# jasonkyuyim/se3_diffusion

Measured on AMD Instinct MI355X. Metric: residues/sec IPA fwd+bwd, higher is better.
Workload: dtype f32

## Files before the change

include/fd_hip.h:

```cpp
#ifndef FD_HIP_H_
#define FD_HIP_H_

#ifdef __cplusplus
extern "C" {
#endif

#define FD_ABI_VERSION 2

const char* fd_last_error(void);
int fd_abi_version(void);
const char* fd_backend(void);
const char* fd_build_flags(void);
long fd_launch_count(void);

typedef struct FdGemmDesc {
  const float* A;
  const float* B;
  float* C;
  int M, N, K;
  long a_rs, a_cs;
  long b_rs, b_cs;
  long ldc;
  int batch, bdiv;
  long a_so, a_si, b_so, b_si, c_so, c_si;
  float alpha;
  int beta;
  const float* bias;
  const float* pair_p;
  const float* pair_q;
  long ld_pair;
  int nres;
  const float* resid;
  long ld_resid;
  const float* gate;
  long ld_gate;
  const float* rowscale;
  int relu;
  int tile;
  int ksplit;
  int mtiles;
  float* a_rowsum;
  const void* b_planes;
  long b_plane_stride;
} FdGemmDesc;

int fd_gemm(const FdGemmDesc* desc, void* stream);
int fd_split_planes(const float* x, long n, void* planes, void* stream);
int fd_gemm_plan(const FdGemmDesc* desc);
int fd_gemm_set_exact_f32(int exact);
int fd_gemm_set_persistent_blocks(int blocks);

int fd_layernorm_fwd(const float* x, long ldx, const float* gamma, const float* beta, const float* rowscale,
                     float* y, long ldy, float* mean, float* rstd, long rows, int C, float eps, void* stream);
int fd_layernorm_bwd(const float* dy, long lddy, const float* x, long ldx, const float* gamma,
                     const float* rowscale, const float* mean, const float* rstd, float* dx, long lddx,
                     int dx_accum, float* dgamma, float* dbeta, long rows, int C, void* stream);
int fd_colsum_acc(const float* X, long ld, long rows, int ncols, float* out, void* stream);
int fd_pair_reduce_acc(const float* X, int nbatch, int n, int C, float* rowsum, float* colsum, long ld_out,
                       void* stream);
int fd_axpby(float* y, const float* x, float a, float b, long n, void* stream);
int fd_add2d(float* dst, long ldd, const float* src, long lds, long rows, int cols, float a, void* stream);
int fd_rowscale(const float* x, long ldx, const float* rs, float* y, long ldy, long rows, int C, void* stream);

#define FD_EDGE_MLP_IMAGE_BYTES (124 * 12288)
int fd_edge_mlp_pack_zb(const float* W40, void* image, void* stream);
int fd_edge_mlp_pack(const float* W1, const float* W2, const float* Wf, long ld, void* image, void* stream);
int fd_edge_mlp_pack_bwd(const float* Wf, const float* W2, const float* W1, long ld, const float* W40, void* image, void* stream);
typedef struct FdEdgeMlpDesc {
  const float* x;
  const void* img;
  const float* p1;
  const float* q1;
  const float* bias2;
  float* save1;
  float* save2;
  const float* pf;
  const float* qf;
  const float* gamma;
  const float* beta;
  const float* rowscale;
  float* y;
  float* mean;
  float* rstd;
  float* out;
  long rows;
  int nres;
  int backward;
  float eps;
  int blocks;
  long ld_pq;
  long ld_pqf;
  float* zb_out;
  const float* zb_bias;
  unsigned* mask1;
  unsigned* mask2;
  const unsigned* gmask1;
  const unsigned* gmask2;
  const float* ln_y;
  const float* ln_mean;
  const float* ln_rstd;
  const float* ln_gamma;
  const float* ln_rowscale;
  float* dy_out;
  float* ln_dgamma;
  float* ln_dbeta;
  const float* dzb;
  unsigned* sched;
  int shape;
} FdEdgeMlpDesc;
#define FD_EDGE_MLP_W8_MIN_ROWS 65536L
#define FD_EDGE_MLP_PAIR_MAX_ROWS 16384L
int fd_edge_mlp(const FdEdgeMlpDesc* desc, void* stream);

#define FD_EDGE_EMBED_IMAGE_BYTES (24 * 12288)
int fd_edge_embed_pack_zb(const float* W40, void* image, void* stream);
int fd_edge_embed_pack(const float* W0, const float* W2, const float* W4, void* image, void* stream);
typedef struct FdEdgeEmbedDesc {
  const long* seq_idx;
  const float* sc_ca;
  const float* idenom;
  const float* dg_lower;
  const float* dg_upper;
  const void* img;
  const float* p;
  const float* q;
  const float* bias2;
  const float* bias3;
  const float* gamma;
  const float* beta;
  const float* rowscale;
  float* h1;
  float* h2;
  float* h3;
  float* mean;
  float* rstd;
  float* out;
  long rows;
  int nres;
  float eps;
  int blocks;
  float* zb_out;
  const float* zb_bias;
// ... 361 lines not shown
```

se3_diffusion_amd/csrc/fd_norm.hip:

```cpp
#include "fd_common.h"
#include "../../include/fd_hip.h"

namespace {

constexpr int MAXC_PER_LANE = 8;

__global__ __launch_bounds__(256) void layernorm_fwd_kernel(
    const float* __restrict__ x, long ldx, const float* __restrict__ gamma, const float* __restrict__ beta,
    const float* __restrict__ rowscale, float* __restrict__ y, long ldy, float* __restrict__ mean_out,
    float* __restrict__ rstd_out, long rows, int C, float eps) {
  const int lane = fd::lane_id(), wave = fd::wave_id();
  const int npl = C / 64;
  for (long row = (long)blockIdx.x * 4 + wave; row < rows; row += (long)gridDim.x * 4) {
    const float* xr = x + row * ldx;
    float v[MAXC_PER_LANE], gm[MAXC_PER_LANE], bt[MAXC_PER_LANE];
    float s = 0.f;
#pragma unroll
    for (int k = 0; k < MAXC_PER_LANE; ++k)
      if (k < npl) { v[k] = xr[lane + 64 * k]; s += v[k]; }
    const float rs = rowscale ? rowscale[row] : 1.f;
#pragma unroll
    for (int k = 0; k < MAXC_PER_LANE; ++k)
      if (k < npl) { gm[k] = gamma[lane + 64 * k]; bt[k] = beta[lane + 64 * k]; }
    const float mean = fd::wave_sum(s) / (float)C;
// ... 246 lines not shown
    }
#pragma unroll
    for (int u = 0; u < LN_U; ++u) {
      const bool ok = row0 + u < rows;
      const float sc = ok ? rs[u] : 0.f;
      const float4 d = make_float4(dv[u].x * sc, dv[u].y * sc, dv[u].z * sc, dv[u].w * sc);
      const float4 xh = make_float4((xv[u].x - m[u]) * rr[u], (xv[u].y - m[u]) * rr[u], (xv[u].z - m[u]) * rr[u],
                                    (xv[u].w - m[u]) * rr[u]);
      const float4 g = make_float4(d.x * gm.x, d.y * gm.y, d.z * gm.z, d.w * gm.w);
      ag.x += d.x * xh.x; ag.y += d.y * xh.y; ag.z += d.z * xh.z; ag.w += d.w * xh.w;
      ab.x += d.x; ab.y += d.y; ab.z += d.z; ab.w += d.w;
      const float s1 = half_wave_sum((g.x + g.y) + (g.z + g.w)) * (1.0f / 128.0f);
      const float s2 = half_wave_sum((g.x * xh.x + g.y * xh.y) + (g.z * xh.z + g.w * xh.w)) * (1.0f / 128.0f);
      if (ok) {
        float4 o;
        o.x = rr[u] * (g.x - s1 - xh.x * s2);
        o.y = rr[u] * (g.y - s1 - xh.y * s2);
        o.z = rr[u] * (g.z - s1 - xh.z * s2);
        o.w = rr[u] * (g.w - s1 - xh.w * s2);
        if (dx_accum) { o.x += old[u].x; o.y += old[u].y; o.z += old[u].z; o.w += old[u].w; }
        *reinterpret_cast<float4*>(dx + (row0 + u) * lddx + 4 * hl) = o;
      }
    }
  }
  if (dgamma) {
    red[0][wave * 2 + half][hl] = ag;
    red[1][wave * 2 + half][hl] = ab;
    __syncthreads();
    const int t = (int)threadIdx.x;
    const int w = t >> 7, ch = t & 127;
    const float* r0 = reinterpret_cast<const float*>(&red[w][0][0]);
    float a = 0.f;
#pragma unroll
    for (int k = 0; k < 8; ++k) a += r0[k * 128 + ch];
    atomicAdd((w == 0 ? dgamma : dbeta) + ch, a);
  }
}

__global__ __launch_bounds__(256) void colsum_kernel(const float* __restrict__ X, long ld, long rows, int ncols,
                                                      float* __restrict__ out) {
  __shared__ float red[4][64];
  const int lane = fd::lane_id(), wave = fd::wave_id();
  for (int c0 = 0; c0 < ncols; c0 += 64) {
    const int c = c0 + lane;
    float acc = 0.f;
    if (c < ncols)
      for (long r = (long)blockIdx.x * 4 + wave; r < rows; r += (long)gridDim.x * 4) acc += X[r * ld + c];
    red[wave][lane] = acc;
    __syncthreads();
    if (wave == 0 && c < ncols) atomicAdd(&out[c], red[0][lane] + red[1][lane] + red[2][lane] + red[3][lane]);
    __syncthreads();
  }
}

__global__ __launch_bounds__(256) void pair_reduce_kernel(const float* __restrict__ X, int n, int C,
                                                          float* __restrict__ rowsum, float* __restrict__ colsum,
                                                          long ld_out) {
  const long bi = blockIdx.x;
  const long b = bi / n;
  const float* xb = X + bi * (long)n * C;
  for (int c = (int)threadIdx.x; c < C; c += (int)blockDim.x) {
    float acc = 0.f;
    for (int j = 0; j < n; ++j) {
      float v = xb[(long)j * C + c];
      acc += v;
      if (colsum) atomicAdd(&colsum[(b * n + j) * ld_out + c], v);
    }
    if (rowsum) rowsum[bi * ld_out + c] += acc;
  }
}

__global__ __launch_bounds__(256) void pair_colsum_kernel(const float* __restrict__ X, int n, int C,
                                                          float* __restrict__ colsum, long ld_out) {
  const long bj = blockIdx.x;
  const long b = bj / n, j = bj % n;
  const float* xb = X + (b * n * (long)n + j) * C;
  for (int c = (int)threadIdx.x; c < C; c += (int)blockDim.x) {
    float acc = 0.f;
    for (int i = 0; i < n; ++i) acc += xb[(long)i * n * C + c];
    colsum[bj * ld_out + c] += acc;
  }
}

constexpr int PR_I = 32, PR_J = 128, PR_C = 32;
__global__ __launch_bounds__(256) void pair_reduce2_kernel(const float* __restrict__ X, int n, int C,
                                                           float* __restrict__ rowsum, float* __restrict__ colsum,
                                                           long ld_out, int nich, int ncc) {
  __shared__ float4 red[PR_I][4][8];
  const int tid = (int)threadIdx.x;
  const int c4 = tid & 7, jg = tid >> 3, wave = tid >> 6;
  int bx = (int)blockIdx.x;
  const int cc = bx % ncc; bx /= ncc;
  const int ic = bx % nich;
  const long b = bx / nich;
  const int j0 = (int)blockIdx.y * PR_J;
  const int c = cc * PR_C + 4 * c4;
  const int i0 = ic * PR_I;
  float4 cs[PR_J / 32];
#pragma unroll
  for (int q = 0; q < PR_J / 32; ++q) cs[q] = make_float4(0.f, 0.f, 0.f, 0.f);
#pragma unroll 4
  for (int il = 0; il < PR_I; ++il) {
    const int i = i0 + il;
    float4 rs = make_float4(0.f, 0.f, 0.f, 0.f);
    if (i < n) {
      const float* xi = X + ((b * n + i) * (long)n) * C + c;
#pragma unroll
      for (int q = 0; q < PR_J / 32; ++q) {
        const int j = j0 + jg + 32 * q;
        if (j < n) {
          const float4 v = *reinterpret_cast<const float4*>(xi + (long)j * C);
          rs.x += v.x; rs.y += v.y; rs.z += v.z; rs.w += v.w;
          cs[q].x += v.x; cs[q].y += v.y; cs[q].z += v.z; cs[q].w += v.w;
        }
      }
    }
    rs.x += fd::lane_xor8(rs.x); rs.y += fd::lane_xor8(rs.y); rs.z += fd::lane_xor8(rs.z); rs.w += fd::lane_xor8(rs.w);
#pragma unroll
    for (int o = 16; o < 64; o <<= 1) {
      rs.x += __shfl_xor(rs.x, o); rs.y += __shfl_xor(rs.y, o); rs.z += __shfl_xor(rs.z, o); rs.w += __shfl_xor(rs.w, o);
    }
    if ((tid & 63) < 8) red[il][wave][c4] = rs;
  }
#pragma unroll
  for (int q = 0; q < PR_J / 32; ++q) {
    const int j = j0 + jg + 32 * q;
    if (j < n) {
      float* o = colsum + (b * n + j) * ld_out + c;
      atomicAdd(o + 0, cs[q].x); atomicAdd(o + 1, cs[q].y); atomicAdd(o + 2, cs[q].z); atomicAdd(o + 3, cs[q].w);
    }
  }
  __syncthreads();
  {
    const int il = tid >> 3, g = tid & 7;
    const int i = i0 + il;
    if (i < n) {
      float4 a = red[il][0][g];
#pragma unroll
      for (int k = 1; k < 4; ++k) {
        const float4 v = red[il][k][g];
        a.x += v.x; a.y += v.y; a.z += v.z; a.w += v.w;
      }
      float* o = rowsum + (b * n + i) * ld_out + cc * PR_C + 4 * g;
      if (gridDim.y == 1) {
        o[0] += a.x; o[1] += a.y; o[2] += a.z; o[3] += a.w;
      } else {
        atomicAdd(o + 0, a.x); atomicAdd(o + 1, a.y); atomicAdd(o + 2, a.z); atomicAdd(o + 3, a.w);
      }
    }
  }
}

__global__ __launch_bounds__(256) void axpby_kernel(float* __restrict__ y, const float* __restrict__ x, float a,
                                                    float b, long n) {
  for (long i = (long)blockIdx.x * 256 + threadIdx.x; i < n; i += (long)gridDim.x * 256) y[i] = a * x[i] + b * y[i];
}

__global__ __launch_bounds__(256) void rowscale_kernel(const float* __restrict__ x, long ldx,
                                                       const float* __restrict__ rs, float* __restrict__ y, long ldy,
                                                       long rows, int C) {
  const long total = rows * C;
  for (long i = (long)blockIdx.x * 256 + threadIdx.x; i < total; i += (long)gridDim.x * 256) {
    long r = i / C;
    int c = (int)(i % C);
    y[r * ldy + c] = x[r * ldx + c] * rs[r];
  }
}

__global__ __launch_bounds__(256) void colsum4_kernel(const float* __restrict__ X, long ld, long rows, int ncols,
                                                       float* __restrict__ out) {
  __shared__ float4 red[4][64];
  const int lane = fd::lane_id(), wave = fd::wave_id();
  const long wg = (long)blockIdx.x * 4 + wave, nw = (long)gridDim.x * 4;
  for (int c0 = 0; c0 < ncols; c0 += 256) {
    const int c = c0 + lane * 4;
    float4 acc0 = make_float4(0.f, 0.f, 0.f, 0.f), acc1 = acc0, acc2 = acc0, acc3 = acc0;
    if (c < ncols) {
      long r = wg;
      for (; r + 3 * nw < rows; r += 4 * nw) {
        const float4 v0 = *reinterpret_cast<const float4*>(X + r * ld + c);
        const float4 v1 = *reinterpret_cast<const float4*>(X + (r + nw) * ld + c);
        const float4 v2 = *reinterpret_cast<const float4*>(X + (r + 2 * nw) * ld + c);
        const float4 v3 = *reinterpret_cast<const float4*>(X + (r + 3 * nw) * ld + c);
        acc0.x += v0.x; acc0.y += v0.y; acc0.z += v0.z; acc0.w += v0.w;
        acc1.x += v1.x; acc1.y += v1.y; acc1.z += v1.z; acc1.w += v1.w;
        acc2.x += v2.x; acc2.y += v2.y; acc2.z += v2.z; acc2.w += v2.w;
        acc3.x += v3.x; acc3.y += v3.y; acc3.z += v3.z; acc3.w += v3.w;
      }
      for (; r < rows; r += nw) {
        const float4 v0 = *reinterpret_cast<const float4*>(X + r * ld + c);
        acc0.x += v0.x; acc0.y += v0.y; acc0.z += v0.z; acc0.w += v0.w;
      }
    }
    float4 s;
    s.x = (acc0.x + acc1.x) + (acc2.x + acc3.x);
    s.y = (acc0.y + acc1.y) + (acc2.y + acc3.y);
    s.z = (acc0.z + acc1.z) + (acc2.z + acc3.z);
    s.w = (acc0.w + acc1.w) + (acc2.w + acc3.w);
    red[wave][lane] = s;
    __syncthreads();
    {
      const int t = (int)threadIdx.x, cc = c0 + t;
      if (cc < ncols) {
        const float* r0 = reinterpret_cast<const float*>(&red[0][0]);
        atomicAdd(&out[cc], (r0[t] + r0[256 + t]) + (r0[512 + t] + r0[768 + t]));
      }
    }
    __syncthreads();
  }
}

__global__ __launch_bounds__(256) void add2d_kernel(float* __restrict__ dst, long ldd, const float* __restrict__ src,
                                                    long lds, long rows, int cols, float a) {
  const long total = rows * cols;
  for (long i = (long)blockIdx.x * 256 + threadIdx.x; i < total; i += (long)gridDim.x * 256) {
    long r = i / cols;
    int c = (int)(i % cols);
    dst[r * ldd + c] += a * src[r * lds + c];
  }
}

}

static int ln_grid(long rows) {
  long g = (rows + 3) / 4;
  return (int)(g < 1 ? 1 : (g > 8192 ? 8192 : g));
}

static bool ln128_ok(const float* p, long ld) { return fd_aligned16(p) && (ld & 3) == 0; }

extern "C" int fd_layernorm_fwd(const float* x, long ldx, const float* gamma, const float* beta,
                                const float* rowscale, float* y, long ldy, float* mean, float* rstd, long rows,
                                int C, float eps, void* stream) {
  FD_CHECK_ARG(C % 64 == 0 && C <= 64 * MAXC_PER_LANE, "fd_layernorm_fwd: C=%d must be a multiple of 64 <= 512", C);
  if (rows == 0) return FD_OK;
  if (C == 128 && ln128_ok(x, ldx) && ln128_ok(y, ldy) && fd_aligned16(gamma) && fd_aligned16(beta)) {
    long g = (rows + 8 * LN_U - 1) / (8 * LN_U);
    int grid = (int)(g < 1 ? 1 : (g > 4096 ? 4096 : g));
    hipLaunchKernelGGL(layernorm_fwd128_kernel, dim3(grid), dim3(256), 0, (hipStream_t)stream, x, ldx, gamma, beta,
                       rowscale, y, ldy, mean, rstd, rows, eps);
    FD_CHECK_LAUNCH("fd_layernorm_fwd(128)");
    return FD_OK;
  }
  hipLaunchKernelGGL(layernorm_fwd_kernel, dim3(ln_grid(rows)), dim3(256), 0, (hipStream_t)stream, x, ldx, gamma,
                     beta, rowscale, y, ldy, mean, rstd, rows, C, eps);
  FD_CHECK_LAUNCH("fd_layernorm_fwd");
  return FD_OK;
}

extern "C" int fd_layernorm_bwd(const float* dy, long lddy, const float* x, long ldx, const float* gamma,
                                const float* rowscale, const float* mean, const float* rstd, float* dx, long lddx,
                                int dx_accum, float* dgamma, float* dbeta, long rows, int C, void* stream) {
  FD_CHECK_ARG(C % 64 == 0 && C <= 64 * MAXC_PER_LANE, "fd_layernorm_bwd: C=%d must be a multiple of 64 <= 512", C);
  FD_CHECK_ARG((dgamma == nullptr) == (dbeta == nullptr), "fd_layernorm_bwd: dgamma/dbeta come together");
  if (rows == 0) return FD_OK;
  if (C == 128 && ln128_ok(x, ldx) && ln128_ok(dy, lddy) && ln128_ok(dx, lddx) && fd_aligned16(gamma)) {
    long g128 = (rows + 8 * LN_U - 1) / (8 * LN_U);
    int grid128 = (int)(g128 < 1 ? 1 : (g128 > 512 ? 512 : g128));
    hipLaunchKernelGGL(layernorm_bwd128_kernel, dim3(grid128), dim3(256), 0, (hipStream_t)stream, dy, lddy, x, ldx,
                       gamma, rowscale, mean, rstd, dx, lddx, dx_accum, dgamma, dbeta, rows);
    FD_CHECK_LAUNCH("fd_layernorm_bwd(128)");
    return FD_OK;
  }
  long g = (rows + 15) / 16;
  int grid = (int)(g < 1 ? 1 : (g > 1024 ? 1024 : g));
  if (ln128_ok(x, ldx) && ln128_ok(dy, lddy) && ln128_ok(dx, lddx) && fd_aligned16(gamma)) {
    if (C <= 256)
      hipLaunchKernelGGL(layernorm_bwd4_kernel<1>, dim3(grid), dim3(256), 0, (hipStream_t)stream, dy, lddy, x, ldx, gamma,
                         rowscale, mean, rstd, dx, lddx, dx_accum, dgamma, dbeta, rows, C);
    else
      hipLaunchKernelGGL(layernorm_bwd4_kernel<2>, dim3(grid), dim3(256), 0, (hipStream_t)stream, dy, lddy, x, ldx, gamma,
                         rowscale, mean, rstd, dx, lddx, dx_accum, dgamma, dbeta, rows, C);
    FD_CHECK_LAUNCH("fd_layernorm_bwd(x4)");
    return FD_OK;
  }
  hipLaunchKernelGGL(layernorm_bwd_kernel, dim3(grid), dim3(256), 0, (hipStream_t)stream, dy, lddy, x, ldx, gamma,
                     rowscale, mean, rstd, dx, lddx, dx_accum, dgamma, dbeta, rows, C);
  FD_CHECK_LAUNCH("fd_layernorm_bwd");
  return FD_OK;
}

extern "C" int fd_colsum_acc(const float* X, long ld, long rows, int ncols, float* out, void* stream) {
  if (rows == 0 || ncols == 0) return FD_OK;
  long g = (rows + 15) / 16;
  int grid = (int)(g < 1 ? 1 : (g > 1024 ? 1024 : g));
  if ((ld & 3) == 0 && (ncols & 3) == 0 && fd_aligned16(X)) {
    hipLaunchKernelGGL(colsum4_kernel, dim3(grid), dim3(256), 0, (hipStream_t)stream, X, ld, rows, ncols, out);
    FD_CHECK_LAUNCH("fd_colsum_acc");
    return FD_OK;
  }
  hipLaunchKernelGGL(colsum_kernel, dim3(grid), dim3(256), 0, (hipStream_t)stream, X, ld, rows, ncols, out);
  FD_CHECK_LAUNCH("fd_colsum_acc");
  return FD_OK;
}

extern "C" int fd_pair_reduce_acc(const float* X, int nbatch, int n, int C, float* rowsum, float* colsum,
                                  long ld_out, void* stream) {
  if (nbatch == 0 || n == 0) return FD_OK;
  if (rowsum && colsum && (C % PR_C) == 0 && fd_aligned16(X)) {
    const int nich = fd_cdiv(n, PR_I), ncc = C / PR_C;
    hipLaunchKernelGGL(pair_reduce2_kernel, dim3(nbatch * nich * ncc, fd_cdiv(n, PR_J)), dim3(256), 0, (hipStream_t)stream,
                       X, n, C, rowsum, colsum, ld_out, nich, ncc);
    FD_CHECK_LAUNCH("fd_pair_reduce_acc(fused)");
    return FD_OK;
  }
  int threads = C >= 256 ? 256 : (C >= 128 ? 128 : 64);
  if (rowsum) {
    hipLaunchKernelGGL(pair_reduce_kernel, dim3(nbatch * n), dim3(threads), 0, (hipStream_t)stream, X, n, C, rowsum,
                       (float*)nullptr, ld_out);
    FD_CHECK_LAUNCH("fd_pair_reduce_acc(row)");
  }
  if (colsum) {
    hipLaunchKernelGGL(pair_colsum_kernel, dim3(nbatch * n), dim3(threads), 0, (hipStream_t)stream, X, n, C, colsum,
                       ld_out);
    FD_CHECK_LAUNCH("fd_pair_reduce_acc(col)");
  }
  return FD_OK;
}

extern "C" int fd_axpby(float* y, const float* x, float a, float b, long n, void* stream) {
  if (n == 0) return FD_OK;
  long g = (n + 255) / 256;
  int grid = (int)(g > 4096 ? 4096 : g);
  hipLaunchKernelGGL(axpby_kernel, dim3(grid), dim3(256), 0, (hipStream_t)stream, y, x, a, b, n);
  FD_CHECK_LAUNCH("fd_axpby");
  return FD_OK;
}

extern "C" int fd_rowscale(const float* x, long ldx, const float* rs, float* y, long ldy, long rows, int C,
                           void* stream) {
  if (rows == 0 || C == 0) return FD_OK;
  long g = (rows * C + 255) / 256;
  int grid = (int)(g > 4096 ? 4096 : g);
  hipLaunchKernelGGL(rowscale_kernel, dim3(grid), dim3(256), 0, (hipStream_t)stream, x, ldx, rs, y, ldy, rows, C);
  FD_CHECK_LAUNCH("fd_rowscale");
  return FD_OK;
}

extern "C" int fd_add2d(float* dst, long ldd, const float* src, long lds, long rows, int cols, float a,
                        void* stream) {
  if (rows == 0 || cols == 0) return FD_OK;
  long g = (rows * cols + 255) / 256;
  int grid = (int)(g > 4096 ? 4096 : g);
  hipLaunchKernelGGL(add2d_kernel, dim3(grid), dim3(256), 0, (hipStream_t)stream, dst, ldd, src, lds, rows, cols, a);
  FD_CHECK_LAUNCH("fd_add2d");
  return FD_OK;
}
```

se3_diffusion_amd/hip.py:

```python
from __future__ import annotations

import ctypes
import os
from ctypes import POINTER, Structure, c_char_p, c_double, c_float, c_int, c_long, c_void_p

import torch

_HERE = os.path.dirname(os.path.abspath(__file__))
LIB_PATH = os.path.join(_HERE, "lib", "libfd_hip.so")


_RAW_STREAM = getattr(torch._C, "_cuda_getCurrentRawStream", None)


class FdError(RuntimeError):
    pass


class FdGemmDesc(Structure):
    _fields_ = [
        ("A", c_void_p), ("B", c_void_p), ("C", c_void_p),
        ("M", c_int), ("N", c_int), ("K", c_int),
        ("a_rs", c_long), ("a_cs", c_long),
        ("b_rs", c_long), ("b_cs", c_long),
# ... 112 lines not shown


class FdPairDwDesc(Structure):
    _fields_ = [("item", FdPairDwItem * PAIR_DW_MAX_ITEMS), ("nitems", c_int), ("rows", c_long), ("blocks", c_int)]


GROUP_DW_MAX_ITEMS = 32


class FdGroupDwItem(Structure):
    __slots__ = ()
    _fields_ = [("A", c_void_p), ("B", c_void_p), ("C", c_void_p), ("a_colsum", c_void_p),
                ("lda", c_int), ("ldb", c_int), ("ldc", c_int), ("n_out", c_int), ("k_in", c_int)]


class FdGroupDwDesc(Structure):
    _fields_ = [("item", FdGroupDwItem * GROUP_DW_MAX_ITEMS), ("nitems", c_int), ("rows", c_long), ("blocks", c_int)]


OPT_WS_DOUBLES = 3 * 4096
OPT_STATE_BYTES = 72


class FdOptState(Structure):
    __slots__ = ()
    _fields_ = [
        ("step", c_long), ("skipped", c_long), ("clipped", c_long), ("nonfinite", c_long),
        ("grad_norm", c_double), ("clip_coef", c_double), ("max_abs", c_double),
        ("bc1", c_float), ("rsqrt_bc2", c_float), ("coef", c_float), ("apply", c_int),
    ]


assert ctypes.sizeof(FdOptState) == OPT_STATE_BYTES


ABI_VERSION = 2


def _ptr(t, off=0):
    if t is None:
        return None
    if isinstance(t, tuple):
        t, off = t
    return t.data_ptr() + t.element_size() * int(off)


def fill_ptrs(desc, **fields):
    tens = []
    for name, t in fields.items():
        if t is None:
            continue
        if type(t) is tuple:
            off = t[1]
            t = t[0]
            setattr(desc, name, t.data_ptr() + t.element_size() * int(off))
        else:
            setattr(desc, name, t.data_ptr())
        tens.append(t)
    return tens


_SIGS = {
    "fd_gemm": "Ss",
    "fd_gemm_plan": "S",
    "fd_split_planes": "plps",
    "fd_gemm_set_exact_f32": "i",
    "fd_gemm_set_persistent_blocks": "i",
    "fd_edge_mlp_pack": "ppplps",
    "fd_edge_mlp": "Ss",
    "fd_edge_mlp_pack_zb": "pps",
    "fd_edge_mlp_pack_bwd": "ppplpps",
    "fd_edge_embed_pack": "pppps",
    "fd_edge_embed": "Ss",
    "fd_edge_embed_pack_zb": "pps",
    "fd_edge_embed_bwd_pack": "ppps",
    "fd_edge_embed_bwd": "Ss",
    "fd_ln_gemm": "Ss",
    "fd_pair_dw": "Ss",
    "fd_group_dw": "Ss",
    "fd_layernorm_fwd": "plpppplpplifs",
    "fd_layernorm_bwd": "plplpppppl" + "ipplis",
    "fd_colsum_acc": "pllips",
    "fd_pair_reduce_acc": "piiippls",
    "fd_axpby": "ppffls",
    "fd_rowscale": "plppllis",
    "fd_add2d": "plpllifs",
    "fd_node_feats": "ppppppiis",
    "fd_node_feats_ld": "ppppppliis",
    "fd_edge_feats": "pppppppppiis",
    "fd_ipa_points_fwd": "pppppppiliiiis",
    "fd_ipa_points_bwd": "pppppppliiiis",
    "fd_ipa_softmax_fwd": "ppppppiis",
    "fd_ipa_attn_fwd": "ppppppppiis",
    "fd_ipa_flash_fwd": "ppppppppppp" + "iiis",
    "fd_ipa_flash_fwd_split": "ppppppppppp" + "iiii" + "ps",
    "fd_ipa_flash_bwd": "pppppppppppp" + "pppppp" + "iis",
    "fd_ipa_flash_bwd_keys": "pppppppp" + "ppp" + "iiis",
    "fd_ipa_opt_bwd_dot": "ppppppp" + "ls",
    "fd_seq_attn_fwd": "ppppfiis",
    "fd_seq_attn_bwd": "pppppfiis",
    "fd_ipa_attn_bwd": "pppppppppppppiis",
    "fd_ipa_softmax_bwd": "ppppppppppiis",
    "fd_ipa_kpts_bwd": "pppppiis",
    "fd_ipa_dz_acc": "ppplis",
    "fd_ipa_opt_fwd": "ppppls",
    "fd_ipa_opt_bwd": "pppppls",
    "fd_ipa_opair_fwd": "pppiis",
    "fd_ipa_opair_bwd": "pppppiis",
    "fd_row_softmax_fwd": "pplii" + "s",
    "fd_row_softmax_bwd": "pplis",
    "fd_split_rigids": "pfpfppplis",
    "fd_bb_update_fwd": "plipppppppp" + "ls",
    "fd_bb_update_bwd": "pppppppppp" + "ls",
    "fd_heads_fwd": "pppp" + "pl" + "ppp" + "pi" + "S" + "ppppppp" + "iis",
    "fd_heads_bwd": "ppppp" + "ppp" + "pi" + "S" + "ppppp" + "ppp" + "iis",
    "fd_backbone_atoms": "ppSppls",
    "fd_igso3_tables": "ppiiippps",
    "fd_sample_ref": "pppppidpls",
    "fd_forward_marginal": "ppppppipdddipppp" + "ls",
    "fd_forward_marginal_batch": "ppppppippdipppp" + "iis",
    "fd_se3_reverse_step": "ppppppiiddpdddiiips",
    "fd_se3_reverse_step_f32": "ppppppiiddpdddiiips",
    "fd_se3_reverse_step_net": "ppppppiiddpdddiiips",
    "fd_sample_advance": "ppppilpipps",
    "fd_sample_record": "ppppp" + "S" + "piili" + "pppp" + "s",
    "fd_dsm_loss": "Ss",
    "fd_adam_step": "pppplffffffs",
    "fd_adam_step_ema": "ppppplfffffffs",
    "fd_grad_stats": "plpps",
    "fd_adam_step_guarded": "pppplddddd" + "i" + "pp" + "s",
    "fd_adam_step_guarded_ema": "ppppplddddd" + "i" + "pp" + "di" + "s",
    "fd_backbone_metrics": "plpiips",
    "fd_aligned_rmsd": "plplpppiipps",
    "fd_tm_search": "plplppp" + "iiiii" + "ppp" + "s",
    "fd_tm_align": "pliplipppp" + "iiii" + "pppp" + "s",
    "fd_dssp_hbonds": "plppiipps",
    "fd_dssp_assign": "plipppiipps",
    "fd_violations": "plppiippppps",
    "fd_cluster_linkage": "pllp" + "iiii" + "ppps",
    "fd_cluster_cut": "pppllp" + "iii" + "d" + "ppps",
    "fd_chain_windows": "pppips",
    "fd_chain_batch": "pppppp" + "ii" + "S" + "ppppp" + "s",
    "fd_mpnn_graph": "pppp" + "li" + "ppp" + "s",
    "fd_mpnn_encoder": "ppp" + "li" + "pp" + "ppppp" + "s",
    "fd_mpnn_decode": "pp" + "ilii" + "pppp" + "pppppp" + "fi" + "pppp" + "s",
    "fd_pdb_count": "plpp" + "ii" + "pp" + "s",
    "fd_pdb_format": "plppp" + "iil" + "pl" + "s",
}
_CT = {"p": c_void_p, "i": c_int, "l": c_long, "f": c_float, "d": c_double, "S": c_void_p, "s": c_void_p}


class FdLib:

    def __init__(self, path: str):
        if not os.path.exists(path):
            raise FdError(
                f"HIP extension not found at {path}. Build it with "
                f"`python -m se3_diffusion_amd.build` (hipcc, gfx950). There is no CPU fallback.")
        self.path = path
        self.cdll = ctypes.CDLL(path)
        for name, (res, args) in {"fd_last_error": (c_char_p, []), "fd_abi_version": (c_int, []), "fd_launch_count": (c_long, []),
                                  "fd_backend": (c_char_p, []), "fd_build_flags": (c_char_p, [])}.items():
            fn = getattr(self.cdll, name)
            fn.restype, fn.argtypes = res, args
        for name, sig in _SIGS.items():
            fn = getattr(self.cdll, name)
# ... 131 lines not shown
```

se3_diffusion_amd/trunk.py:

```python
from __future__ import annotations

import math

import numpy as np
import torch

from . import hip, ops
from .trace import rng
from . import network as nw
from .network import CS, CZ, TD, H, _lin_grads
from .ops import empty, zeros, mv, lib
from .options import opts

EH = 384
CE = 128


def bb_update_fwd(P, b, n3, dmask, quat, trans, R):
    pre = f"score_model.trunk.bb_update_{b}.linear"
    dev = n3
    upd = empty((R, 6), dev); q2 = empty((R, 4), dev); t2 = empty((R, 3), dev)
    lib().call("fd_bb_update_fwd", n3, CS, CS, dmask, P[f"{pre}.weight"], P[f"{pre}.bias"], quat, trans, upd, q2, t2, R)
    return q2, t2, dict(n3=n3, dmask=dmask, quat=quat, upd=upd, R=R)

# ... 48 lines not shown
        key = ("et_fold", pre)
        if key not in cache:
            Wi, bi = P[f"{pre}.initial_embed.weight"], P[f"{pre}.initial_embed.bias"]
            Wcat = torch.cat([W1[:, CZ:CZ + CE], W1[:, CZ + CE:], Wf[:, CZ:CZ + CE], Wf[:, CZ + CE:]], 0).contiguous()
            Wfold = empty((LDT, CS), Wi)
            ops.linear(mv(Wcat), mv(Wi.t().contiguous()), None, mv(Wfold), LDT, CS, CE)
            bvec = torch.cat([torch.zeros_like(P[f"{pre}.trunk.0.bias"]), P[f"{pre}.trunk.0.bias"],
                              torch.zeros_like(P[f"{pre}.final_layer.bias"]), P[f"{pre}.final_layer.bias"]]).contiguous()
            bfold = empty((1, LDT), Wi)
            ops.linear(mv(bi.view(1, CE)), mv(Wcat), bvec, mv(bfold), 1, LDT, CE)
            cache[key] = (Wfold, bfold.view(-1))
        Wfold, bfold = cache[key]
        PQ = empty((R, LDT), Wfold)
        if n3_ln is not None:
            t_in, g_in, b_in, rs_in, _, n3_out = n3_ln
            ops.ln_linear(mv(t_in), g_in, b_in, mv(Wfold), bfold, mv(PQ), R, LDT, CS, ln_rowscale=rs_in, ln_out=mv(n3_out))
        else:
            ops.linear(mv(n3), mv(Wfold), bfold, mv(PQ), R, LDT, CS)
        return PQ[:, 0:], PQ[:, EH:], PQ[:, 2 * EH:], PQ[:, 2 * EH + CZ:], LDT, None
    dev = n3
    e = empty((R, CE), dev)
    ops.linear(mv(n3), mv(P[f"{pre}.initial_embed.weight"]), P[f"{pre}.initial_embed.bias"], mv(e), R, CE, CS)
    P1 = empty((R, EH), dev); Q1 = empty((R, EH), dev); Pf = empty((R, CZ), dev); Qf = empty((R, CZ), dev)
    ops.linear(mv(e), (W1, CZ, EH), None, mv(P1), R, EH, CE)
    ops.linear(mv(e), (W1, CZ + CE, EH), P[f"{pre}.trunk.0.bias"], mv(Q1), R, EH, CE)
    ops.linear(mv(e), (Wf, CZ, EH), None, mv(Pf), R, CZ, CE)
    ops.linear(mv(e), (Wf, CZ + CE, EH), P[f"{pre}.final_layer.bias"], mv(Qf), R, CZ, CE)
    return P1, Q1, Pf, Qf, 0, e


def edge_transition_pair(P, b, terms, n3, z, emask, B, N, save=True, cache=None, zb_next=None):
    pre = f"score_model.trunk.edge_transition_{b}"
    dev = z
    Pn = B * N * N
    P1, Q1, Pf, Qf, ld, e = terms
    kw = {}
    zb = None
    use_zb = (opts.zb_from_edge and zb_next is not None and zb_next[0].is_contiguous() and zb_next[0].data_ptr() % 16 == 0
              and zb_next[1].data_ptr() % 16 == 0)
    img = _edge_mlp_image(P, pre, cache, W40=zb_next[0] if use_zb else None)
    z2 = empty((Pn, CZ), dev)
    if save:
        h1 = empty((Pn, EH), dev); h2 = empty((Pn, EH), dev); y = empty((Pn, CZ), dev)
        mean = empty((Pn,), dev); rstd = empty((Pn,), dev)
        mh1 = empty((Pn, 12), dev, torch.int32); mh2 = empty((Pn, 12), dev, torch.int32)
        kw = dict(save1=h1, save2=h2, y=y, mean=mean, rstd=rstd, mask1=mh1, mask2=mh2)
    if use_zb:
        zb = empty((Pn, nw.ZB), dev)
        kw.update(zb_out=zb, zb_bias=zb_next[1])
    ops.edge_mlp(z, img, z2, Pn, N, p1=P1, q1=Q1, bias2=P[f"{pre}.trunk.2.bias"], pf=Pf, qf=Qf, ld_pq=ld, ld_pqf=ld,
                 gamma=P[f"{pre}.layer_norm.weight"], beta=P[f"{pre}.layer_norm.bias"], rowscale=emask, **kw)
    if not save:
        return z2, None, zb
    return z2, dict(n3=n3, z=z, e=e, h1=h1, h2=h2, y=y, mean=mean, rstd=rstd, emask=emask, B=B, N=N,
                    mh1=mh1, mh2=mh2, h2_has_z=True), zb


def edge_transition_fwd_unfused(P, b, n3, z, emask, B, N):
    pre = f"score_model.trunk.edge_transition_{b}"
    dev = z
    R, Pn = B * N, B * N * N
    W1, Wf = P[f"{pre}.trunk.0.weight"], P[f"{pre}.final_layer.weight"]
    e = empty((R, CE), dev)
    ops.linear(mv(n3), mv(P[f"{pre}.initial_embed.weight"]), P[f"{pre}.initial_embed.bias"], mv(e), R, CE, CS)
    P1 = empty((R, EH), dev); Q1 = empty((R, EH), dev)
    ops.linear(mv(e), (W1, CZ, EH), None, mv(P1), R, EH, CE)
    ops.linear(mv(e), (W1, CZ + CE, EH), P[f"{pre}.trunk.0.bias"], mv(Q1), R, EH, CE)
    h1 = empty((Pn, EH), dev)
    ops.linear(mv(z), (W1, 0, EH), None, mv(h1), Pn, EH, CZ, relu=True, pair=(P1, Q1, EH, N))
    h2 = empty((Pn, EH), dev)
    ops.linear(mv(h1), mv(P[f"{pre}.trunk.2.weight"]), P[f"{pre}.trunk.2.bias"], mv(h2), Pn, EH, EH, relu=True)
    Pf = empty((R, CZ), dev); Qf = empty((R, CZ), dev)
    ops.linear(mv(e), (Wf, CZ, EH), None, mv(Pf), R, CZ, CE)
    ops.linear(mv(e), (Wf, CZ + CE, EH), P[f"{pre}.final_layer.bias"], mv(Qf), R, CZ, CE)
    y = empty((Pn, CZ), dev)
    ops.linear(mv(h2), mv(Wf), None, mv(y), Pn, CZ, EH)
    ops.linear(mv(z), (Wf, 0, EH), None, mv(y), Pn, CZ, CZ, pair=(Pf, Qf, CZ, N), beta=True)
    z2 = empty((Pn, CZ), dev); mean = empty((Pn,), dev); rstd = empty((Pn,), dev)
    ops.layernorm(mv(y), P[f"{pre}.layer_norm.weight"], P[f"{pre}.layer_norm.bias"], mv(z2), Pn, CZ, rowscale=emask,
                  save=(mean, rstd))
    return z2, dict(n3=n3, z=z, e=e, h1=h1, h2=h2, y=y, mean=mean, rstd=rstd, emask=emask, B=B, N=N)


def _node_terms_bwd(G, dx, C, W, gW, bias, e, de, B, N, accumulate):
    R = B * N
    dP = zeros((R, C), e); dQ = zeros((R, C), e)
    lib().call("fd_pair_reduce_acc", dx, B, N, C, dP, dQ, C)
    wi, wj = (gW, CZ, EH), (gW, CZ + CE, EH)
    if ops.queue_dw_ok(mv(dP), mv(e), wi, R, C, CE) and ops.queue_dw_ok(mv(dQ), mv(e), wj, R, C, CE):
        ops.queue_dw(mv(dP), mv(e), wi, R, C, CE)
        ops.queue_dw(mv(dQ), mv(e), wj, R, C, CE, db=G[bias])
    else:
        def _grads():
            ops.linear_dw(mv(dP), mv(e), wi, R, C, CE)
            ops.linear_dw(mv(dQ), mv(e), wj, R, C, CE)
            ops.bias_grad(mv(dQ), G[bias], R, C)
        ops.side(_grads, (dP, dQ, e), R)
    ops.linear_dx(mv(dP), (W, CZ, EH), mv(de), R, C, CE, beta=accumulate)
    ops.linear_dx(mv(dQ), (W, CZ + CE, EH), mv(de), R, C, CE, beta=True)


def edge_transition_bwd(P, G, b, sv, dz2, dz, dn3, dzb_next=None, flush_behind_launch=False):
    pre = f"score_model.trunk.edge_transition_{b}"
    B, N = sv["B"], sv["N"]
    R, Pn = B * N, B * N * N
    dev = sv["z"]
    L = lib()
    W1, W2, Wf = P[f"{pre}.trunk.0.weight"], P[f"{pre}.trunk.2.weight"], P[f"{pre}.final_layer.weight"]
    gW1, gWf = G[f"{pre}.trunk.0.weight"], G[f"{pre}.final_layer.weight"]
    z, e, h1, h2 = sv["z"], sv["e"], sv["h1"], sv["h2"]
    fused = sv.get("mh1") is not None and (fused_edge() or bool(sv.get("h2_has_z")))
    h2_has_z = bool(sv.get("h2_has_z"))
    assert fused or not h2_has_z, "a fused edge-transition forward needs the fused backward (its h2 save carries z)"
    fused_ln = fused and opts.fused_ln_bwd and (dzb_next is None or dzb_next[1].is_contiguous())
    grouped_dw = fused and opts.grouped_pair_dw
    dy = empty((Pn, CZ), dev)
    de = empty((R, CE), dev)

    def ln_bwd(dz2):
        if dzb_next is not None:
            acc = dz2 is not None
            dz2 = dz2 if acc else empty((Pn, CZ), dev)
            L.call("fd_ipa_dz_acc", dzb_next[0], dzb_next[1].contiguous(), dz2, Pn, int(acc))
        if flush_behind_launch:
            ops.flush_dw()
        ops.layernorm_bwd(mv(dz2), mv(sv["y"]), P[f"{pre}.layer_norm.weight"], sv["mean"], sv["rstd"], mv(dy), Pn, CZ,
                          rowscale=sv["emask"], dgamma=G[f"{pre}.layer_norm.weight"], dbeta=G[f"{pre}.layer_norm.bias"])

    def final_layer_grads():
        if not grouped_dw:
            def _grads_y():
                ops.linear_dw(mv(dy), mv(h2), mv(gWf), Pn, CZ, EH)
                if not h2_has_z:
                    ops.linear_dw(mv(dy), mv(z), (gWf, 0, EH), Pn, CZ, CZ)
            ops.side(_grads_y, (dy, h2, z), Pn)
        _node_terms_bwd(G, dy, CZ, Wf, gWf, f"{pre}.final_layer.bias", e, de, B, N, accumulate=False)

    if fused:
        dh2 = empty((Pn, EH), dev); dh1 = empty((Pn, EH), dev)
        dx_args = dict(save1=dh2, save2=dh1, backward=True, gmask1=sv["mh2"], gmask2=sv["mh1"])
    if fused_ln:
        img = ops.edge_mlp_pack_bwd(Wf, W2, W1, W40=dzb_next[1] if dzb_next is not None else None)
        ops.edge_mlp(dz2, img, dz, Pn, N, ln_y=sv["y"], ln_mean=sv["mean"], ln_rstd=sv["rstd"],
                     ln_gamma=P[f"{pre}.layer_norm.weight"], ln_rowscale=sv["emask"], dy_out=dy,
                     ln_dgamma=G[f"{pre}.layer_norm.weight"], ln_dbeta=G[f"{pre}.layer_norm.bias"],
                     dzb=dzb_next[0] if dzb_next is not None else None, **dx_args)
        if flush_behind_launch:
            ops.flush_dw()
        final_layer_grads()
    elif fused:
        ln_bwd(dz2)
        final_layer_grads()
        ops.edge_mlp(dy, _edge_mlp_image(P, pre, None, backward=True), dz, Pn, N, **dx_args)
    else:
        ln_bwd(dz2)
        final_layer_grads()
        ops.linear_dx(mv(dy), (Wf, 0, EH), mv(dz), Pn, CZ, CZ)
        dh2 = empty((Pn, EH), dev)
        ops.linear_dx(mv(dy), mv(Wf), mv(dh2), Pn, CZ, EH, gate=mv(h2))
        _lin_grads(G, f"{pre}.trunk.2.weight", f"{pre}.trunk.2.bias", mv(dh2), mv(h1), Pn, EH, EH)
        dh1 = empty((Pn, EH), dev)
        ops.linear_dx(mv(dh2), mv(W2), mv(dh1), Pn, EH, EH, gate=mv(h1))
    if grouped_dw:
        gW2, gb2 = G[f"{pre}.trunk.2.weight"], G[f"{pre}.trunk.2.bias"]
        items = [dict(A=(dh2, 0, EH), B=(h1, CZ * j, EH), C=(gW2, CZ * j, EH), colsum=gb2 if j == 0 else None)
                 for j in range(3)]
        items.append(dict(A=(dh1, 0, EH), B=(z, 0, CZ), C=(gW1, 0, EH)))
        it = dict(A=(h2, 0, EH), B=(dy, 0, CZ), C=(gWf, 0, EH), trans=True)
        if not h2_has_z:
            it["A_add"] = (z, 0, CZ)
        items.append(it)
        nblk = opts.pair_dw_blocks if ops.side_active(dh2, Pn) else 0
        ops.side(lambda: ops.pair_dw(items, Pn, blocks=nblk), (dh2, dh1, h1, h2, z, dy), Pn)
    else:
        if fused:
            _lin_grads(G, f"{pre}.trunk.2.weight", f"{pre}.trunk.2.bias", mv(dh2), mv(h1), Pn, EH, EH)
        ops.side(lambda: ops.linear_dw(mv(dh1), mv(z), (gW1, 0, EH), Pn, EH, CZ), (dh1, z), Pn)
    del dh2
    _node_terms_bwd(G, dh1, EH, W1, gW1, f"{pre}.trunk.0.bias", e, de, B, N, accumulate=True)
    if not fused:
        ops.linear_dx(mv(dh1), (W1, 0, EH), mv(dz), Pn, EH, CZ, beta=True)
    _lin_grads(G, f"{pre}.initial_embed.weight", f"{pre}.initial_embed.bias", mv(de), mv(sv["n3"]), R, CE, CS)
    ops.linear_dx(mv(de), mv(P[f"{pre}.initial_embed.weight"]), mv(dn3), R, CE, CS, beta=True)


_HC = {}


def head_const(conf_key=(0.1, 0.1, 20.0, 0.1, 1.5, 1000), device=None):
    so3 = conf_key[6] if len(conf_key) > 6 else None
    cached = so3 is not None and device is not None
    conf_key = tuple(conf_key[:6]) + ((str(device),) if cached else ())
    store = so3.__dict__.setdefault("_fd_head_const", {}) if cached else _HC
    if conf_key not in store:
        cs, min_b, max_b, min_s, max_s, L = conf_key[:6]
        n = np.array([-0.525, 1.363, 0.000]); ca = np.zeros(3); c = np.array([1.526, -0.000, -0.000])
        cb = np.array([-0.529, -0.774, -1.205]); o = np.array([0.627, 1.062, 0.000])
        ex = c - ca
        ey = ca - n
        exn = ex / np.linalg.norm(ex)
        eyn = ey - np.dot(ey, exn) * exn
        eyn = eyn / np.linalg.norm(eyn)
        ez = np.cross(exn, eyn)
        Rd = np.stack([exn, eyn, ez], 1)
        hc = hip.FdHeadConst()
        for i, v in enumerate(np.concatenate([n, ca, c, cb, o]).astype(np.float32)):
            hc.atoms[i] = float(v)
        for i, v in enumerate(Rd.astype(np.float32).reshape(-1)):
            hc.Rd[i] = float(v)
        for i, v in enumerate(c.astype(np.float32)):
            hc.td[i] = float(v)
        hc.coord_scale = cs
        hc.exp_max_sigma = float(np.exp(max_s))
        hc.exp_min_sigma = float(np.exp(min_s))
        hc.min_b, hc.max_b, hc.L = min_b, max_b, L
        if cached:
            tab, om = so3.device_score_norms(device), so3.device_tables(device)[1]
            assert tab.shape[1] == om.numel()
            hc.score_norms, hc.omega_grid, hc.n_omega = tab.data_ptr(), om.data_ptr(), om.numel()
            hc._tables = (tab, om)
        store[conf_key] = hc
    return store[conf_key]


_SG = {}


def head_tables(dconf, device):
    num_sigma = dconf[7] if len(dconf) > 7 else 1000
    return head_const(dconf, device), sigma_grid(device, dconf[3], dconf[4], num_sigma)


def sigma_grid(device, min_sigma=0.1, max_sigma=1.5, num_sigma=1000):
    key = (str(device), min_sigma, max_sigma, num_sigma)
    if key not in _SG:
        t = np.linspace(0.0, 1.0, num_sigma)
        g = np.log(t * np.exp(max_sigma) + (1 - t) * np.exp(min_sigma))
        _SG[key] = torch.tensor(g, dtype=torch.float64, device=device)
    return _SG[key]


def heads_fwd(P, node, quat, trans, feats, B, N, dconf, sc_ca_out=None):
    tp = "score_model.torsion_pred"
    dev = node
    R = B * N
    h1 = empty((R, CS), dev); h2 = empty((R, CS), dev); u = empty((R, 2), dev)
    ops.linear(mv(node), mv(P[f"{tp}.linear_1.weight"]), P[f"{tp}.linear_1.bias"], mv(h1), R, CS, CS, relu=True)
    ops.linear(mv(h1), mv(P[f"{tp}.linear_2.weight"]), P[f"{tp}.linear_2.bias"], mv(h2), R, CS, CS, resid=mv(node))
    ops.linear(mv(h2), mv(P[f"{tp}.linear_final.weight"]), P[f"{tp}.linear_final.bias"], mv(u), R, 2, CS)
    hc, sg = head_tables(dconf, dev.device)
    rot = empty((B, N, 3), dev, torch.float64); ts = empty((B, N, 3), dev); rig = empty((B, N, 7), dev)
    psi = empty((B, N, 2), dev); a37 = empty((B, N, 37, 3), dev); a14 = empty((B, N, 14, 3), dev)
    gt = feats["torsion_angles_sin_cos"]
    tt = feats["t"].float().contiguous()
    lib().call("fd_heads_fwd", feats["rigids_t"], quat, trans, u, (gt, 4), 14, feats["fixed_mask"], feats["res_mask"],
               tt, sg, sg.numel(), hc, rot, ts, rig, psi, a37, a14, sc_ca_out, B, N)
    out = dict(psi=psi, rot_score=rot, trans_score=ts, rigids=rig, atom37=a37, atom14=a14)
    return out, dict(node=node, h1=h1, h2=h2, u=u, quat=quat, trans=trans, psi=psi, t=tt, hc=hc, sg=sg, B=B, N=N)


def heads_bwd(P, G, sv, feats, d_out, dnode):
    tp = "score_model.torsion_pred"
# ... 259 lines not shown
```

Baseline: 175,600.

## Fuse pair row/col reductions for dy and dh1 into one slab kernel

```diff
diff --git a/include/fd_hip.h b/include/fd_hip.h
--- a/include/fd_hip.h
+++ b/include/fd_hip.h
@@ -58,6 +58,8 @@
 int fd_colsum_acc(const float* X, long ld, long rows, int ncols, float* out, void* stream);
 int fd_pair_reduce_acc(const float* X, int nbatch, int n, int C, float* rowsum, float* colsum, long ld_out,
                        void* stream);
+int fd_pair_reduce2_acc(const float* X1, int C1, const float* X2, int C2, int nbatch, int n, float* rowsum1,
+                        float* colsum1, float* rowsum2, float* colsum2, long ld_out1, long ld_out2, void* stream);
 int fd_axpby(float* y, const float* x, float a, float b, long n, void* stream);
 int fd_add2d(float* dst, long ldd, const float* src, long lds, long rows, int cols, float a, void* stream);
 int fd_rowscale(const float* x, long ldx, const float* rs, float* y, long ldy, long rows, int C, void* stream);
diff --git a/se3_diffusion_amd/csrc/fd_norm.hip b/se3_diffusion_amd/csrc/fd_norm.hip
--- a/se3_diffusion_amd/csrc/fd_norm.hip
+++ b/se3_diffusion_amd/csrc/fd_norm.hip
@@ -352,72 +352,95 @@
   }
 }
 
-constexpr int PR_I = 32, PR_J = 128, PR_C = 32;
-__global__ __launch_bounds__(256) void pair_reduce2_kernel(const float* __restrict__ X, int n, int C,
-                                                           float* __restrict__ rowsum, float* __restrict__ colsum,
-                                                           long ld_out, int nich, int ncc) {
-  __shared__ float4 red[PR_I][4][8];
+constexpr int PR_I = 32, PR_J = 128, PR_S = 128, PR_T = 8, PR_Q = PR_J / 8;
+template <bool FULL_J>
+__global__ __launch_bounds__(256, 2) void pair_reduce_slab_kernel(
+    const float* __restrict__ X1, int C1, float* __restrict__ rowsum1, float* __restrict__ colsum1, long ld1,
+    const float* __restrict__ X2, int C2, float* __restrict__ rowsum2, float* __restrict__ colsum2, long ld2,
+    int n, int nich, int ns1, int ns) {
+  __shared__ float4 red[PR_T][8][32];
   const int tid = (int)threadIdx.x;
-  const int c4 = tid & 7, jg = tid >> 3, wave = tid >> 6;
+  const int c4 = tid & 31, jg = tid >> 5;
   int bx = (int)blockIdx.x;
-  const int cc = bx % ncc; bx /= ncc;
+  int s = bx % ns; bx /= ns;
   const int ic = bx % nich;
   const long b = bx / nich;
-  const int j0 = (int)blockIdx.y * PR_J;
-  const int c = cc * PR_C + 4 * c4;
-  const int i0 = ic * PR_I;
-  float4 cs[PR_J / 32];
-#pragma unroll
-  for (int q = 0; q < PR_J / 32; ++q) cs[q] = make_float4(0.f, 0.f, 0.f, 0.f);
-#pragma unroll 4
-  for (int il = 0; il < PR_I; ++il) {
-    const int i = i0 + il;
-    float4 rs = make_float4(0.f, 0.f, 0.f, 0.f);
-    if (i < n) {
-      const float* xi = X + ((b * n + i) * (long)n) * C + c;
-#pragma unroll
-      for (int q = 0; q < PR_J / 32; ++q) {
-        const int j = j0 + jg + 32 * q;
-        if (j < n) {
-          const float4 v = *reinterpret_cast<const float4*>(xi + (long)j * C);
-          rs.x += v.x; rs.y += v.y; rs.z += v.z; rs.w += v.w;
-          cs[q].x += v.x; cs[q].y += v.y; cs[q].z += v.z; cs[q].w += v.w;
+  const bool second = s >= ns1;
+  const float* X = second ? X2 : X1;
+  const int C = second ? C2 : C1;
+  float* rowsum = second ? rowsum2 : rowsum1;
+  float* colsum = second ? colsum2 : colsum1;
+  const long ld_out = second ? ld2 : ld1;
+  if (second) s -= ns1;
+  const int j0 = (int)blockIdx.y * PR_J, i0 = ic * PR_I;
+  const int c0 = s * PR_S;
+  const float* lds = reinterpret_cast<const float*>(&red[0][0][0]);
+  float4 cs[PR_Q];
+#pragma unroll
+  for (int q = 0; q < PR_Q; ++q) cs[q] = make_float4(0.f, 0.f, 0.f, 0.f);
+  for (int it0 = i0; it0 < i0 + PR_I && it0 < n; it0 += PR_T) {
+#pragma unroll 1
+    for (int it = 0; it < PR_T; ++it) {
+      float4 rs = make_float4(0.f, 0.f, 0.f, 0.f);
+      const int i = it0 + it;
+      if (i < n) {
+        const float* xi = X + ((b * n + i) * (long)n + j0 + jg) * C + c0 + 4 * c4;
+        float4 v[PR_Q];
+#pragma unroll
+        for (int q = 0; q < PR_Q; ++q)
+          v[q] = (FULL_J || j0 + jg + 8 * q < n) ? *reinterpret_cast<const float4*>(xi + (long)(8 * q) * C)
+                                                 : make_float4(0.f, 0.f, 0.f, 0.f);
+#pragma unroll
+        for (int q = 0; q < PR_Q; ++q) {
+          rs.x += v[q].x; rs.y += v[q].y; rs.z += v[q].z; rs.w += v[q].w;
+          cs[q].x += v[q].x; cs[q].y += v[q].y; cs[q].z += v[q].z; cs[q].w += v[q].w;
         }
       }
-    }
-    rs.x += fd::lane_xor8(rs.x); rs.y += fd::lane_xor8(rs.y); rs.z += fd::lane_xor8(rs.z); rs.w += fd::lane_xor8(rs.w);
-#pragma unroll
-    for (int o = 16; o < 64; o <<= 1) {
-      rs.x += __shfl_xor(rs.x, o); rs.y += __shfl_xor(rs.y, o); rs.z += __shfl_xor(rs.z, o); rs.w += __shfl_xor(rs.w, o);
-    }
-    if ((tid & 63) < 8) red[il][wave][c4] = rs;
-  }
-#pragma unroll
-  for (int q = 0; q < PR_J / 32; ++q) {
-    const int j = j0 + jg + 32 * q;
-    if (j < n) {
-      float* o = colsum + (b * n + j) * ld_out + c;
-      atomicAdd(o + 0, cs[q].x); atomicAdd(o + 1, cs[q].y); atomicAdd(o + 2, cs[q].z); atomicAdd(o + 3, cs[q].w);
-    }
-  }
-  __syncthreads();
-  {
-    const int il = tid >> 3, g = tid & 7;
-    const int i = i0 + il;
-    if (i < n) {
-      float4 a = red[il][0][g];
-#pragma unroll
-      for (int k = 1; k < 4; ++k) {
-        const float4 v = red[il][k][g];
-        a.x += v.x; a.y += v.y; a.z += v.z; a.w += v.w;
-      }
-      float* o = rowsum + (b * n + i) * ld_out + cc * PR_C + 4 * g;
-      if (gridDim.y == 1) {
-        o[0] += a.x; o[1] += a.y; o[2] += a.z; o[3] += a.w;
-      } else {
-        atomicAdd(o + 0, a.x); atomicAdd(o + 1, a.y); atomicAdd(o + 2, a.z); atomicAdd(o + 3, a.w);
-      }
-    }
+      red[it][jg][c4] = rs;
+    }
+    __syncthreads();
+    constexpr int RK = PR_T * PR_S / 256;
+    float a[RK], old[RK];
+    float* o[RK];
+#pragma unroll
+    for (int k = 0; k < RK; ++k) {
+      const int idx = k * 256 + tid, il = idx / PR_S, ch = idx % PR_S;
+      const int i = it0 + il < n ? it0 + il : n - 1;
+      o[k] = rowsum + (b * n + i) * ld_out + c0 + ch;
+      const float* r = lds + il * (8 * PR_S) + ch;
+      a[k] = r[0];
+#pragma unroll
+      for (int g = 1; g < 8; ++g) a[k] += r[g * PR_S];
+    }
+    if (gridDim.y == 1) {
+#pragma unroll
+      for (int k = 0; k < RK; ++k) old[k] = *o[k];
+#pragma unroll
+      for (int k = 0; k < RK; ++k)
+        if (it0 + (k * 256 + tid) / PR_S < n) *o[k] = old[k] + a[k];
+    } else {
+#pragma unroll
+      for (int k = 0; k < RK; ++k)
+        if (it0 + (k * 256 + tid) / PR_S < n) atomicAdd(o[k], a[k]);
+    }
+    __syncthreads();
+  }
+#pragma unroll
+  for (int round = 0; round < PR_Q / 8; ++round) {
+#pragma unroll
+    for (int q = 0; q < 8; ++q) red[q][jg][c4] = cs[round * 8 + q];
+    __syncthreads();
+#pragma unroll 8
+    for (int k = 0; k < 64 * PR_S / 256; ++k) {
+      const int idx = k * 256 + tid, r = idx / PR_S, ch = idx % PR_S;
+      const int j = j0 + (r & 7) + 8 * (round * 8 + (r >> 3));
+      if (j < n) {
+        float* o = colsum + (b * n + j) * ld_out + c0 + ch;
+        if (nich == 1) *o += lds[idx];
+        else atomicAdd(o, lds[idx]);
+      }
+    }
+    __syncthreads();
   }
 }
 
@@ -564,14 +587,28 @@
   return FD_OK;
 }
 
+static bool pair_reduce_slab_launch(const float* X1, int C1, float* rowsum1, float* colsum1, long ld1, const float* X2,
+                                    int C2, float* rowsum2, float* colsum2, long ld2, int nbatch, int n,
+                                    hipStream_t stream) {
+  if (!rowsum1 || !colsum1 || C1 <= 0 || (C1 % PR_S) != 0 || !fd_aligned16(X1)) return false;
+  if (X2 && (!rowsum2 || !colsum2 || C2 <= 0 || (C2 % PR_S) != 0 || !fd_aligned16(X2))) return false;
+  const int nich = fd_cdiv(n, PR_I), ns1 = C1 / PR_S, ns = ns1 + (X2 ? C2 / PR_S : 0);
+  const dim3 grid(nbatch * nich * ns, fd_cdiv(n, PR_J));
+  if ((n % PR_J) == 0)
+    hipLaunchKernelGGL(HIP_KERNEL_NAME(pair_reduce_slab_kernel<true>), grid, dim3(256), 0, stream, X1, C1, rowsum1, colsum1,
+                       ld1, X2, C2, rowsum2, colsum2, ld2, n, nich, ns1, ns);
+  else
+    hipLaunchKernelGGL(HIP_KERNEL_NAME(pair_reduce_slab_kernel<false>), grid, dim3(256), 0, stream, X1, C1, rowsum1, colsum1,
+                       ld1, X2, C2, rowsum2, colsum2, ld2, n, nich, ns1, ns);
+  return true;
+}
+
 extern "C" int fd_pair_reduce_acc(const float* X, int nbatch, int n, int C, float* rowsum, float* colsum,
                                   long ld_out, void* stream) {
   if (nbatch == 0 || n == 0) return FD_OK;
-  if (rowsum && colsum && (C % PR_C) == 0 && fd_aligned16(X)) {
-    const int nich = fd_cdiv(n, PR_I), ncc = C / PR_C;
-    hipLaunchKernelGGL(pair_reduce2_kernel, dim3(nbatch * nich * ncc, fd_cdiv(n, PR_J)), dim3(256), 0, (hipStream_t)stream,
-                       X, n, C, rowsum, colsum, ld_out, nich, ncc);
-    FD_CHECK_LAUNCH("fd_pair_reduce_acc(fused)");
+  if (pair_reduce_slab_launch(X, C, rowsum, colsum, ld_out, nullptr, 0, nullptr, nullptr, 0, nbatch, n,
+                              (hipStream_t)stream)) {
+    FD_CHECK_LAUNCH("fd_pair_reduce_acc(slab)");
     return FD_OK;
   }
   int threads = C >= 256 ? 256 : (C >= 128 ? 128 : 64);
@@ -586,6 +623,21 @@
     FD_CHECK_LAUNCH("fd_pair_reduce_acc(col)");
   }
   return FD_OK;
+}
+
+extern "C" int fd_pair_reduce2_acc(const float* X1, int C1, const float* X2, int C2, int nbatch, int n, float* rowsum1,
+                                   float* colsum1, float* rowsum2, float* colsum2, long ld_out1, long ld_out2,
+                                   void* stream) {
+  FD_CHECK_ARG(X1 != nullptr, "fd_pair_reduce2_acc: X1 is null");
+  if (nbatch == 0 || n == 0) return FD_OK;
+  if (pair_reduce_slab_launch(X1, C1, rowsum1, colsum1, ld_out1, X2, C2, rowsum2, colsum2, ld_out2, nbatch, n,
+                              (hipStream_t)stream)) {
+    FD_CHECK_LAUNCH("fd_pair_reduce2_acc");
+    return FD_OK;
+  }
+  int rc = fd_pair_reduce_acc(X1, nbatch, n, C1, rowsum1, colsum1, ld_out1, stream);
+  if (rc == FD_OK && X2) rc = fd_pair_reduce_acc(X2, nbatch, n, C2, rowsum2, colsum2, ld_out2, stream);
+  return rc;
 }
 
 extern "C" int fd_axpby(float* y, const float* x, float a, float b, long n, void* stream) {
diff --git a/se3_diffusion_amd/hip.py b/se3_diffusion_amd/hip.py
--- a/se3_diffusion_amd/hip.py
+++ b/se3_diffusion_amd/hip.py
@@ -218,6 +218,7 @@
     "fd_layernorm_bwd": "plplpppppl" + "ipplis",
     "fd_colsum_acc": "pllips",
     "fd_pair_reduce_acc": "piiippls",
+    "fd_pair_reduce2_acc": "pipiiipppplls",
     "fd_axpby": "ppffls",
     "fd_rowscale": "plppllis",
     "fd_add2d": "plpllifs",
diff --git a/se3_diffusion_amd/trunk.py b/se3_diffusion_amd/trunk.py
--- a/se3_diffusion_amd/trunk.py
+++ b/se3_diffusion_amd/trunk.py
@@ -154,10 +154,13 @@
     return z2, dict(n3=n3, z=z, e=e, h1=h1, h2=h2, y=y, mean=mean, rstd=rstd, emask=emask, B=B, N=N)
 
 
-def _node_terms_bwd(G, dx, C, W, gW, bias, e, de, B, N, accumulate):
+def _node_terms_bwd(G, dx, C, W, gW, bias, e, de, B, N, accumulate, reduced=None):
     R = B * N
-    dP = zeros((R, C), e); dQ = zeros((R, C), e)
-    lib().call("fd_pair_reduce_acc", dx, B, N, C, dP, dQ, C)
+    if reduced is not None:
+        dP, dQ = reduced
+    else:
+        dP = zeros((R, C), e); dQ = zeros((R, C), e)
+        lib().call("fd_pair_reduce_acc", dx, B, N, C, dP, dQ, C)
     wi, wj = (gW, CZ, EH), (gW, CZ + CE, EH)
     if ops.queue_dw_ok(mv(dP), mv(e), wi, R, C, CE) and ops.queue_dw_ok(mv(dQ), mv(e), wj, R, C, CE):
         ops.queue_dw(mv(dP), mv(e), wi, R, C, CE)
@@ -186,6 +189,7 @@
     assert fused or not h2_has_z, "a fused edge-transition forward needs the fused backward (its h2 save carries z)"
     fused_ln = fused and opts.fused_ln_bwd and (dzb_next is None or dzb_next[1].is_contiguous())
     grouped_dw = fused and opts.grouped_pair_dw
+    red_h1 = None
     dy = empty((Pn, CZ), dev)
     de = empty((R, CE), dev)
 
@@ -199,14 +203,14 @@
         ops.layernorm_bwd(mv(dz2), mv(sv["y"]), P[f"{pre}.layer_norm.weight"], sv["mean"], sv["rstd"], mv(dy), Pn, CZ,
                           rowscale=sv["emask"], dgamma=G[f"{pre}.layer_norm.weight"], dbeta=G[f"{pre}.layer_norm.bias"])
 
-    def final_layer_grads():
+    def final_layer_grads(reduced=None):
         if not grouped_dw:
             def _grads_y():
                 ops.linear_dw(mv(dy), mv(h2), mv(gWf), Pn, CZ, EH)
                 if not h2_has_z:
                     ops.linear_dw(mv(dy), mv(z), (gWf, 0, EH), Pn, CZ, CZ)
             ops.side(_grads_y, (dy, h2, z), Pn)
-        _node_terms_bwd(G, dy, CZ, Wf, gWf, f"{pre}.final_layer.bias", e, de, B, N, accumulate=False)
+        _node_terms_bwd(G, dy, CZ, Wf, gWf, f"{pre}.final_layer.bias", e, de, B, N, accumulate=False, reduced=reduced)
 
     if fused:
         dh2 = empty((Pn, EH), dev); dh1 = empty((Pn, EH), dev)
@@ -219,7 +223,10 @@
                      dzb=dzb_next[0] if dzb_next is not None else None, **dx_args)
         if flush_behind_launch:
             ops.flush_dw()
-        final_layer_grads()
+        red_y = (zeros((R, CZ), e), zeros((R, CZ), e))
+        red_h1 = (zeros((R, EH), e), zeros((R, EH), e))
+        L.call("fd_pair_reduce2_acc", dh1, EH, dy, CZ, B, N, *red_h1, *red_y, EH, CZ)
+        final_layer_grads(red_y)
     elif fused:
         ln_bwd(dz2)
         final_layer_grads()
@@ -249,7 +256,7 @@
             _lin_grads(G, f"{pre}.trunk.2.weight", f"{pre}.trunk.2.bias", mv(dh2), mv(h1), Pn, EH, EH)
         ops.side(lambda: ops.linear_dw(mv(dh1), mv(z), (gW1, 0, EH), Pn, EH, CZ), (dh1, z), Pn)
     del dh2
-    _node_terms_bwd(G, dh1, EH, W1, gW1, f"{pre}.trunk.0.bias", e, de, B, N, accumulate=True)
+    _node_terms_bwd(G, dh1, EH, W1, gW1, f"{pre}.trunk.0.bias", e, de, B, N, accumulate=True, reduced=red_h1)
     if not fused:
         ops.linear_dx(mv(dh1), (W1, 0, EH), mv(dz), Pn, EH, CZ, beta=True)
     _lin_grads(G, f"{pre}.initial_embed.weight", f"{pre}.initial_embed.bias", mv(de), mv(sv["n3"]), R, CE, CS)
```

Result: no change. 176,700 (median of 6 runs) (+0.6%).
